# geonuklee/slam-toolkit

Hardware: NVIDIA B200
Metric: orb_extract_match_stereo_frames_per_s (higher is better)
Workload: dtype u8

## Files before the change

### slam-toolkit_b200/csrc/sfe_extract.cu

```cuda
#include <cuda_fp16.h>

#include <algorithm>
#include <cmath>
#include <mutex>
#include <type_traits>

#include "sfe_extract.cuh"

namespace sfe {

__device__ __forceinline__ uint32_t ldg_word_at(const uint8_t *p) {
    const uintptr_t a = (uintptr_t)p;
    const uint32_t *w = (const uint32_t *)(a & ~(uintptr_t)3);
    return __funnelshift_r(__ldg(w), __ldg(w + 1), (uint32_t)(a & 3) * 8);
}

__device__ __forceinline__ uint32_t dp4a_u8u8(uint32_t a, uint32_t b, uint32_t c) {
    uint32_t d;
    asm("dp4a.u32.u32 %0, %1, %2, %3;" : "=r"(d) : "r"(a), "r"(b), "r"(c));
    return d;
}
__device__ __forceinline__ uint32_t dp2a_lo(uint32_t a, uint32_t b, uint32_t c) {
    uint32_t d;
    asm("dp2a.lo.u32.u32 %0, %1, %2, %3;" : "=r"(d) : "r"(a), "r"(b), "r"(c));
// ... 892 lines not shown
        if (t.x0 == 0 || t.x0 + kBlurTileW + 3 > w) {
            for (int it = tid; it < IH * 6; it += 256) {
                const int r = (it * 10923) >> 16, k = it - r * 6;
                const int x = k < 3 ? k - 3 : w + (k - 3);
                const int c = x - x_first, sc = (k < 3 ? -x : 2 * w - 2 - x) - x_first;
                if (c >= 0 && c < IWW * 4 && sc >= 0) in8[r * IWW * 4 + c] = in8[r * IWW * 4 + sc];
            }
            __syncthreads();
        }
        if (t.y0 == 0 || t.y0 + kBlurTileH + 3 > h) {
            for (int it = tid; it < 6 * IWW; it += 256) {
                const int k = (it * (65536 / IWW + 1)) >> 16, j = it - k * IWW;
                const int y = k < 3 ? k - 3 : h + (k - 3);
                const int r = y - y_first, sr = (k < 3 ? -y : 2 * h - 2 - y) - y_first;
                if (r >= 0 && r < IH && sr >= 0) in32[r * IWW + j] = in32[sr * IWW + j];
            }
            __syncthreads();
        }
    } else {
        int pitch;
        const uint8_t *src = level_pixels(S, l, img, pitch);
        constexpr int kFirst = kBlurLead / 4 - 1, kWords = kBlurTileW / 4 + 2;
        for (int it = tid; it < IH * kWords; it += 256) {
            const int r = (it * (65536 / kWords + 1)) >> 16, j = kFirst + it - r * kWords;
            int yy = y_first + r;
            if ((unsigned)yy >= (unsigned)h) yy = reflect101(yy, h);
            const uint8_t *row = src + (size_t)yy * pitch;
            const int x = x_first + 4 * j;
            uint32_t v;
            if (x >= 0 && x + 8 <= w) {
                v = ldg_word_at(row + x);
            } else {
                v = __ldg(row + reflect101(x, w)) | (uint32_t)__ldg(row + reflect101(x + 1, w)) << 8 |
                    (uint32_t)__ldg(row + reflect101(x + 2, w)) << 16 | (uint32_t)__ldg(row + reflect101(x + 3, w)) << 24;
            }
            in32[r * IWW + j] = v;
        }
        __syncthreads();
    }
    constexpr uint32_t kTapLo = 18u | 34u << 8 | 48u << 16 | 56u << 24, kTapHi = 48u | 34u << 8 | 18u << 16;
    for (int it = tid; it < (IH / 2) * (kBlurTileW / 4); it += 256) {
        const int rp = it >> 5, g = it & 31;
        uint32_t hsum[2][4];
#pragma unroll
        for (int q = 0; q < 2; q++) {
            const uint32_t *wp = &in32[(2 * rp + q) * IWW + g + (kBlurLead / 4 - 1)];
            const uint32_t w0 = wp[0], w1 = wp[1], w2 = wp[2];
            hsum[q][0] = dp4a_u8u8(__byte_perm(w0, w1, 0x4321), kTapLo, dp4a_u8u8(__byte_perm(w1, w2, 0x4321), kTapHi, 0));
            hsum[q][1] = dp4a_u8u8(__byte_perm(w0, w1, 0x5432), kTapLo, dp4a_u8u8(__byte_perm(w1, w2, 0x5432), kTapHi, 0));
            hsum[q][2] = dp4a_u8u8(__byte_perm(w0, w1, 0x6543), kTapLo, dp4a_u8u8(__byte_perm(w1, w2, 0x6543), kTapHi, 0));
            hsum[q][3] = dp4a_u8u8(w1, kTapLo, dp4a_u8u8(w2, kTapHi, 0));
        }
        *(uint4 *)&hb[rp * kBlurTileW + 4 * g] =
            make_uint4(__byte_perm(hsum[0][0], hsum[1][0], 0x5410), __byte_perm(hsum[0][1], hsum[1][1], 0x5410),
                       __byte_perm(hsum[0][2], hsum[1][2], 0x5410), __byte_perm(hsum[0][3], hsum[1][3], 0x5410));
    }
    __syncthreads();
    uint8_t *dst = S.blur + (size_t)slot * S.blur_stride + L.blur_off;
    const int cg = tid & 31, r0 = (tid >> 5) * 4;
    const int gx = t.x0 + 4 * cg;
    if (gx >= w) return;
    uint4 pr[5];
#pragma unroll
    for (int p = 0; p < 5; p++) pr[p] = *(const uint4 *)&hb[(r0 / 2 + p) * kBlurTileW + 4 * cg];
    constexpr uint32_t kEvenA = 18u | 34u << 8 | 48u << 16 | 56u << 24, kEvenB = 48u | 34u << 8 | 18u << 16;
    constexpr uint32_t kOddA = 18u << 8 | 34u << 16 | 48u << 24, kOddB = 56u | 48u << 8 | 34u << 16 | 18u << 24;
#pragma unroll
    for (int k = 0; k < 4; k++) {
        const int gy = t.y0 + r0 + k;
        if (gy >= h) break;
        const int p = k >> 1;
        uint32_t v[4];
#pragma unroll
        for (int c = 0; c < 4; c++) {
            const uint32_t a0 = (&pr[p].x)[c], a1 = (&pr[p + 1].x)[c], a2 = (&pr[p + 2].x)[c], a3 = (&pr[p + 3].x)[c];
            v[c] = (k & 1) ? dp2a_hi(a3, kOddB, dp2a_lo(a2, kOddB, dp2a_hi(a1, kOddA, dp2a_lo(a0, kOddA, 32768u))))
                           : dp2a_hi(a3, kEvenB, dp2a_lo(a2, kEvenB, dp2a_hi(a1, kEvenA, dp2a_lo(a0, kEvenA, 32768u))));
        }
        *(uint32_t *)(dst + (size_t)gy * L.blur_pitch + gx) =
            __byte_perm(__byte_perm(v[0], v[1], 0x0062), __byte_perm(v[2], v[3], 0x0062), 0x5410);
    }
}

__device__ const signed char g_pattern[1024] = {
#include "orb_pattern_data.inc"
};

__device__ __forceinline__ float fast_atan2_deg(float y, float x) {
    constexpr float s = (float)(180.0 / 3.1415926535897932384626433832795);
    constexpr float p1 = 0.9997878412794807f * s, p3 = -0.3258083974640975f * s, p5 = 0.1555786518463281f * s,
                    p7 = -0.04432655554792128f * s;
    const float ax = fabsf(x), ay = fabsf(y);
    const float eps = 2.220446049250313e-16f;
    float a, c, c2;
    if (ax >= ay) {
        c = __fdiv_rn(ay, __fadd_rn(ax, eps));
        c2 = __fmul_rn(c, c);
        a = __fmul_rn(__fadd_rn(__fmul_rn(__fadd_rn(__fmul_rn(__fadd_rn(__fmul_rn(p7, c2), p5), c2), p3), c2), p1), c);
    } else {
        c = __fdiv_rn(ax, __fadd_rn(ay, eps));
        c2 = __fmul_rn(c, c);
        a = __fsub_rn(90.f, __fmul_rn(__fadd_rn(__fmul_rn(__fadd_rn(__fmul_rn(__fadd_rn(__fmul_rn(p7, c2), p5), c2), p3), c2), p1), c));
    }
    if (x < 0) a = __fsub_rn(180.f, a);
    if (y < 0) a = __fsub_rn(360.f, a);
    return a;
}

constexpr int kUmax[16] = {15, 15, 15, 15, 14, 14, 14, 13, 13, 12, 11, 10, 9, 8, 6, 3};
constexpr bool disc_is_symmetric() {
    for (int u = 0; u < 16; u++)
        for (int v = 0; v < 16; v++)
            if ((u <= kUmax[v]) != (v <= kUmax[u])) return false;
    return true;
}
static_assert(disc_is_symmetric(), "IC_Angle disc must be symmetric");
struct DiscTable {
    uint32_t u[16][8], in[16][8];
};
constexpr DiscTable make_disc_table() {
    DiscTable t{};
    for (int v = 0; v < 16; v++)
        for (int j = 0; j < 8; j++)
            for (int k = 0; k < 4; k++) {
                const int u = -kHalfPatch + 4 * j + k, au = u < 0 ? -u : u;
                if (au <= kUmax[v]) {
                    t.u[v][j] |= (uint32_t)(u & 0xFF) << (8 * k);
                    t.in[v][j] |= 1u << (8 * k);
                }
            }
    return t;
}
__device__ const DiscTable g_disc = make_disc_table();

__device__ __forceinline__ int dp4a_u8s8(uint32_t pix, uint32_t w, int acc) {
    int d;
    asm("dp4a.u32.s32 %0, %1, %2, %3;" : "=r"(d) : "r"(pix), "r"(w), "r"(acc));
    return d;
}

constexpr int kPatchR = 18;
constexpr int kPatchRows = 2 * kPatchR + 1, kPatchWords = 10;
constexpr signed char kPatternHost[1024] = {
#include "orb_pattern_data.inc"
};
constexpr bool pattern_within_patch() {
    for (int i = 0; i < 512; i++) {
        const int px = kPatternHost[2 * i], py = kPatternHost[2 * i + 1];
        if (4 * (px * px + py * py) >= (2 * kPatchR + 1) * (2 * kPatchR + 1)) return false;
    }
    return true;
}
static_assert(pattern_within_patch(), "a rotated pattern point could round outside the staged window");
#ifndef SFE_KP_PER_WARP
#define SFE_KP_PER_WARP 8
#endif
constexpr int kKpPerWarp = SFE_KP_PER_WARP;

constexpr int kIcBoxW = 48, kIcBoxH = 2 * kHalfPatch + 1, kBdBoxW = 64, kBdBoxH = kPatchRows;
constexpr int kIcBytes = 1536, kWinBytes = kIcBytes + 2432;
struct OrientMaps {
    CUtensorMap ic[kMaxLevels], ic_l0b;
    CUtensorMap bd[kMaxLevels];
};

template <bool kTma>
__global__ void __launch_bounds__(256, 5) orient_describe_kernel(ImgSet S, OutSet O, int kp_per_warp, const __grid_constant__ OrientMaps M) {
    __shared__ float2 pat[16 * 32];
    __shared__ __align__(128) uint8_t win_all[8][kTma ? kWinBytes : kPatchRows * kPatchWords * 4];
    __shared__ uint64_t bars[8];
    pdl_enter();
    const int tid = threadIdx.x, lane = tid & 31, warp = tid >> 5, img = blockIdx.y, slot = slot_of(S, img);
    uint32_t *patch = (uint32_t *)win_all[warp];
    uint32_t phase = 0;
    if (kTma && lane == 0) mbar_init(&bars[warp], 1);
    for (int i = tid; i < 512; i += 256) {
        const int byte = i >> 4, s = i & 15;
        pat[s * 32 + byte] = make_float2((float)g_pattern[2 * i], (float)g_pattern[2 * i + 1]);
    }
    const int wj = lane & 7, wr0 = 2 * (lane >> 3);
    auto ic_row = [wr0](int t) { return 8 * (t >> 1) + (t & 1) + wr0; };
    uint32_t wu[8], win[8];
#pragma unroll
    for (int t = 0; t < 8; t++) {
        const int r = ic_row(t), adv = r < 31 ? (r < kHalfPatch ? kHalfPatch - r : r - kHalfPatch) : 0;
        wu[t] = r < 31 ? __ldg(&g_disc.u[adv][wj]) : 0u;
        win[t] = r < 31 ? __ldg(&g_disc.in[adv][wj]) : 0u;
    }
    __syncthreads();
    const int cnt = lane < S.nlevels ? min(S.kp_count[slot * S.nlevels + lane], S.lv[lane].kp_cap) : 0;
    int inc = cnt;
#pragma unroll
    for (int o = 1; o < kMaxLevels; o <<= 1) {
        const int u = __shfl_up_sync(0xffffffffu, inc, o);
        if (lane >= o) inc += u;
    }
    const int total = __shfl_sync(0xffffffffu, inc, kMaxLevels - 1);
    const bool set_a = img < S.split;
    const int oi = set_a ? img : img - S.split;
    if (blockIdx.x == 0 && tid == 0) {
        (set_a ? O.n_a : O.n_b)[oi] = min(total, O.cap);
        if (total > O.cap) atomicOr(&S.flags[slot], kFlagOutOverflow);
    }
    const int g0 = (blockIdx.x * 8 + warp) * kp_per_warp;
    for (int g = g0; g < g0 + kp_per_warp; g++) {
        if (g >= total || g >= O.cap) return;
        const int l = __popc(__ballot_sync(0xffffffffu, lane < S.nlevels && inc <= g));
        const int local = g - __shfl_sync(0xffffffffu, inc - cnt, min(l, 31));
        const LevelPlan &L = S.lv[l];
        const uint32_t v = S.kpst[(size_t)slot * S.kpst_stride + L.kp_off + local];
        const int x = (v & 0xFFF) + kBorder, y = ((v >> 12) & 0xFFF) + kBorder;
        int pitch;
        const uint8_t *lvl = level_pixels(S, l, img, pitch);
        int m10 = 0, m01 = 0;
        const int xl = x - kPatchR, xb0 = xl & ~15;
        if (kTma) {
            const int xi = x - kHalfPatch, xi0 = xi & ~15;
            __syncwarp();
            if (lane == 0) {
                mbar_expect_tx(&bars[warp], kIcBoxW * kIcBoxH + kBdBoxW * kBdBoxH);
                const bool sa = img < S.split;
                const CUtensorMap *mi = l == 0 ? (sa ? &M.ic[0] : &M.ic_l0b) : &M.ic[l];
                tma_load_3d(win_all[warp], mi, &bars[warp], xi0, y - kHalfPatch, l == 0 ? S.in_z0 + (sa ? img : img - S.split) : slot);
                tma_load_3d(win_all[warp] + kIcBytes, &M.bd[l], &bars[warp], xb0, y - kPatchR, slot);
            }
            mbar_wait(&bars[warp], phase);
            phase ^= 1;
            const int o = xi - xi0;
            const uint32_t *w0 = (const uint32_t *)(win_all[warp] + (o & ~3) + 4 * wj);
            const uint32_t sh8 = (uint32_t)(o & 3) * 8;
#pragma unroll
            for (int t = 0; t < 8; t++) {
                const int r = ic_row(t);
                if (r < 31) {
                    const uint32_t *wp = w0 + r * (kIcBoxW / 4);
                    const uint32_t px = __funnelshift_r(wp[0], wp[1], sh8);
                    m10 = dp4a_u8s8(px, wu[t], m10);
                    m01 += (r - kHalfPatch) * dp4a_u8s8(px, win[t], 0);
                }
            }
        } else {
            const uint8_t *r0p = lvl + (size_t)(y - kHalfPatch) * pitch + (x - kHalfPatch + 4 * wj);
#pragma unroll
            for (int t = 0; t < 8; t++) {
                const int r = ic_row(t);
                if (r < 31) {
                    const uint8_t *rp = r0p + (size_t)r * pitch;
                    const uint32_t *wp = (const uint32_t *)((uintptr_t)rp & ~(uintptr_t)3);
                    const uint32_t px = __funnelshift_r(__ldg(wp), __ldg(wp + 1), ((uint32_t)(uintptr_t)rp & 3) * 8);
                    m10 = dp4a_u8s8(px, wu[t], m10);
                    m01 += (r - kHalfPatch) * dp4a_u8s8(px, win[t], 0);
                }
            }
        }
#pragma unroll
        for (int o = 16; o > 0; o >>= 1) {
            m01 += __shfl_xor_sync(0xffffffffu, m01, o);
            m10 += __shfl_xor_sync(0xffffffffu, m10, o);
        }
        const float angle = fast_atan2_deg((float)m01, (float)m10);
        float a = 0.f, b = 0.f;
        if (lane == 0) {
            const float factor_pi = (float)(3.1415926535897932384626433832795 / 180.0);
            const float rad = __fmul_rn(angle, factor_pi);
            double sn, cs;
            sincos((double)rad, &sn, &cs);
            a = (float)cs;
            b = (float)sn;
        }
        a = __shfl_sync(0xffffffffu, a, 0);
        b = __shfl_sync(0xffffffffu, b, 0);
        const uint8_t *pc;
        int wpitch;
        if (kTma) {
            wpitch = kBdBoxW;
            pc = win_all[warp] + kIcBytes + kPatchR * kBdBoxW + (xl - xb0) + kPatchR;
        } else {
            const int bp = L.blur_pitch;
            const uint8_t *bl = S.blur + (size_t)slot * S.blur_stride + L.blur_off;
            const int al = xl & 3;
            __syncwarp();
            if (lane < 3 * kPatchWords) {
                const int rs = lane / kPatchWords, c = lane - rs * kPatchWords;
                const uint32_t *src = (const uint32_t *)(bl + (size_t)(y - kPatchR + rs) * bp + (xl - al)) + c;
                uint32_t *dst = patch + rs * kPatchWords + c;
#pragma unroll
                for (int r = rs; r < kPatchRows; r += 3, src += 3 * (bp >> 2), dst += 3 * kPatchWords) *dst = __ldg(src);
            }
            __syncwarp();
            wpitch = kPatchWords * 4;
            pc = (const uint8_t *)patch + kPatchR * (kPatchWords * 4) + kPatchR + al;
        }
        uint32_t byte = 0;
#pragma unroll
        for (int k = 0; k < 8; k++) {
            int tv[2];
#pragma unroll
            for (int s = 0; s < 2; s++) {
                const float2 pp = pat[(2 * k + s) * 32 + lane];
                const int ry = __float2int_rn(__fadd_rn(__fmul_rn(pp.x, b), __fmul_rn(pp.y, a)));
                const int rx = __float2int_rn(__fsub_rn(__fmul_rn(pp.x, a), __fmul_rn(pp.y, b)));
                tv[s] = pc[ry * wpitch + rx];
            }
            byte |= (uint32_t)(tv[0] < tv[1]) << k;
        }
        uint8_t *desc = (set_a ? O.desc_a : O.desc_b) + ((size_t)oi * O.cap + g) * 32;
        desc[lane] = (uint8_t)byte;
        if (lane == 0) {
            sfe_keypoint kp;
            kp.x = (float)x;
            kp.y = (float)y;
            if (l != 0) {
                kp.x = __fmul_rn(kp.x, L.scale);
                kp.y = __fmul_rn(kp.y, L.scale);
            }
            kp.size = L.size;
            kp.angle = angle;
            kp.response = (float)(v >> 24);
            kp.octave = l;
            kp.class_id = -1;
            (set_a ? O.kps_a : O.kps_b)[(size_t)oi * O.cap + g] = kp;
        }
    }
}

}

using namespace sfe;

enum { kStagePyramid, kStageFast, kStageQuadtree, kStageBlur, kStageDescribe, kStageStereo, kStageTrack, kNumStages };
constexpr int kOctreeSmemCand = 3072;
constexpr int kComputeStreams = 4;
constexpr int kMaxChunks = 16;

struct sfe_extractor {
    int device = 0;
    cudaStream_t stream = nullptr;
    cudaStream_t s_h2d = nullptr, s_d2h = nullptr;
    cudaStream_t extra[kComputeStreams - 1] = {};
    int n_compute = 3;
    cudaStream_t aux[3] = {nullptr, nullptr, nullptr};
    cudaEvent_t ev_fork[3] = {}, ev_join[3] = {};
    int dev_split = 3;
    bool split_small = false;
    int octree_ctas = 0;
    int sm_count = 148;
    bool piped_now = false;
    bool orient_tma = true;
    bool overlap_tail = true;
    bool tail_pending = false;
    int overlap_blur = 2;
    cudaEvent_t ev_start = nullptr;
    bool async_dev = false;
    cudaEvent_t ev_in[kMaxChunks] = {}, ev_done[kMaxChunks] = {};
    int chunks_override = 0;
    bool trace = false;
    cudaEvent_t tr_ev[3 * kMaxChunks + 1] = {};
    sfe_extractor_params prm{};
    float scale[kMaxLevels], inv_scale[kMaxLevels], sigma2[kMaxLevels], inv_sigma2[kMaxLevels];
    int quota[kMaxLevels];
    int max_images = 0;
    int w = 0, h = 0;
    LevelPlan lv[kMaxLevels];
    FastPlan fast{};
    alignas(64) TmaMaps fast_maps{}, blur_maps{}, pyr_maps{};
    alignas(64) OrientMaps orient_maps{};
    int pyr_box_w = 0, pyr_box_h = 0;
    bool tma_plan_ok = false, tma_disabled = false, tma_now = false;
    const void *l0_key[2] = {nullptr, nullptr};
    size_t l0_geom[4] = {0, 0, 0, 0};
    int pitch0 = 0;
    std::vector<SegRec> segs;
    int seg_level_start[kMaxLevels + 1] = {};
    DevBuf<SegRec> d_segs;
    size_t fast_smem = 0, pyr_smem = 0;
    int pyr_wide_h[kMaxLevels] = {};
    std::vector<TilePlan> tiles;
    size_t pyr_stride = 0, blur_stride = 0;
    int cand_stride = 0, kpst_stride = 0, max_cand = 0, max_nodes = 0;
    size_t octree_smem = 0;
    int octree_smem_cand = 0, octree_slots = 0, octree_cand_override = 0;
    struct GraphEntry {
        uint64_t plan_gen = 0;
        int frames = 0, cap = 0, stereo = 0, seen = 0;
        double sp[3] = {0, 0, 0};
        const void *ptr[7] = {};
        cudaGraphExec_t exec = nullptr;
        int64_t launches = 0;
        uint64_t used = 0;
    };
    std::vector<GraphEntry> graphs;
    uint64_t plan_gen = 0, graph_clock = 0;
    bool use_graphs = true;
    bool use_pdl = true;
    bool octree_ff = true;
    bool pdl_now = false;
    bool octree_wide = false;
    int cand_floor[kMaxLevels] = {};
    int cand_cap_override = 0;
    DevBuf<uint8_t> d_octree_scratch;
    DevBuf<uint8_t> d_pyr, d_blur, d_in, d_l0, d_desc;
    DevBuf<uint32_t> d_cand, d_kpst;
    DevBuf<int> d_counts;
    DevBuf<TilePlan> d_tiles;
    DevBuf<uint2> d_xtab, d_ytab;
    DevBuf<sfe_keypoint> d_kps;
    DevBuf<int32_t> d_nout, d_sidx, d_sdist, d_tidx, d_tdist;
    std::vector<int> h_flags;
    int *h_flags_pinned = nullptr;
    uint8_t *h_stage = nullptr;
    size_t h_stage_bytes = 0;
    bool use_copy_kernel = true;
    int64_t launches = 0;
    bool profiling = false;
    cudaEvent_t prof_ev[kNumStages + 1] = {};
    bool prof_pending = false, prof_has_stereo = false, prof_has_track = false;
    TrackScratch track;
    double stage_ms[kNumStages] = {};
    int64_t stage_calls = 0;
    ImgSet last{};
    int last_count = 0;
};

static inline int cv_round_f(float v) { return (int)nearbyintf(v); }

static inline void prof_mark(sfe_extractor *ex, int i) {
    if (ex->profiling) cudaEventRecord(ex->prof_ev[i], ex->stream);
}

static void build_tables(sfe_extractor *ex) {
    const int nl = ex->prm.nlevels;
// ... 422 lines not shown
            SFE_CUDA(cudaFuncSetAttribute(octree_kernel<false>, cudaFuncAttributeMaxDynamicSharedMemorySize, (int)ex->octree_smem));
            SFE_CUDA(cudaFuncSetAttribute(octree_kernel<true>, cudaFuncAttributeMaxDynamicSharedMemorySize, (int)ex->octree_smem));
            granted[ex->device & 63] = ex->octree_smem;
        }
    }
    int *scratch_next = ex->d_counts.p + (size_t)ex->max_images * nl * 2;
    auto launch_octree = [&](cudaStream_t so, int level0, int level_n, int ctas) {
        const int items = level_n * count;
        const int grid = ctas > 0 ? std::min(items, ctas) : items;
        const int threads = nl * count <= ex->sm_count / 2 ? 1024 : 256;
        if (ex->octree_wide)
            launch_k(octree_kernel<true>, grid, threads, ex->octree_smem, so, ex->pdl_now, S, count, level0, level_n, ex->octree_smem_cand,
                     ex->max_cand, ex->max_nodes, ex->d_octree_scratch.p, ex->octree_slots, scratch_next);
        else
            launch_k(octree_kernel<false>, grid, threads, ex->octree_smem, so, ex->pdl_now, S, count, level0, level_n, ex->octree_smem_cand,
                     ex->max_cand, ex->max_nodes, ex->d_octree_scratch.p, ex->octree_slots, scratch_next);
        ex->launches++;
    };
    const bool fork_ok = !ex->profiling && !ex->piped_now && st == ex->stream;
    const bool split = fork_ok && has_cells && ex->split_small && count <= kSplitMaxImages && nl >= 3;
    if (split) {
        launch_pyr(1);
        cudaStream_t sa = ex->aux[2];
        SFE_CUDA(cudaEventRecord(ex->ev_fork[2], st));
        SFE_CUDA(cudaStreamWaitEvent(sa, ex->ev_fork[2], 0));
        if (int rc = launch_fast(ex, sa, S, count, 0, 2)) return rc;
        launch_octree(sa, 0, 2, 0);
        SFE_CUDA(cudaEventRecord(ex->ev_join[2], sa));
        for (int l = 2; l < nl; l++) launch_pyr(l);
        cudaStream_t sb = ex->aux[0];
        SFE_CUDA(cudaEventRecord(ex->ev_fork[0], st));
        SFE_CUDA(cudaStreamWaitEvent(sb, ex->ev_fork[0], 0));
        if (ex->tma_now)
            blur_kernel<true><<<dim3((unsigned)ex->tiles.size(), count), 256, 0, sb>>>(S, ex->d_tiles.p, ex->blur_maps);
        else
            blur_kernel<false><<<dim3((unsigned)ex->tiles.size(), count), 256, 0, sb>>>(S, ex->d_tiles.p, ex->blur_maps);
        SFE_CUDA(cudaEventRecord(ex->ev_join[0], sb));
        if (int rc = launch_fast(ex, st, S, count, 2, nl)) return rc;
        launch_octree(st, 2, nl - 2, 0);
        SFE_CUDA(cudaStreamWaitEvent(st, ex->ev_join[2], 0));
        SFE_CUDA(cudaStreamWaitEvent(st, ex->ev_join[0], 0));
        ex->launches += 3;
    } else {
        for (int l = 1; l < nl; l++) launch_pyr(l);
        prof_mark(ex, 1);
        if (has_cells) {
            const int si = 0;
            const bool fork = ex->overlap_blur && fork_ok, late = ex->overlap_blur == 2;
            cudaStream_t sb = fork ? ex->aux[si] : st;
            auto launch_blur = [&]() {
                if (ex->tma_now)
                    blur_kernel<true><<<dim3((unsigned)ex->tiles.size(), count), 256, 0, sb>>>(S, ex->d_tiles.p, ex->blur_maps);
                else
                    blur_kernel<false><<<dim3((unsigned)ex->tiles.size(), count), 256, 0, sb>>>(S, ex->d_tiles.p, ex->blur_maps);
            };
            auto fork_blur = [&]() -> int {
                SFE_CUDA(cudaEventRecord(ex->ev_fork[si], st));
                SFE_CUDA(cudaStreamWaitEvent(sb, ex->ev_fork[si], 0));
                launch_blur();
                SFE_CUDA(cudaEventRecord(ex->ev_join[si], sb));
                return SFE_OK;
            };
            if (fork && !late)
                if (int rc = fork_blur()) return rc;
            if (int rc = launch_fast(ex, st, S, count)) return rc;
            prof_mark(ex, 2);
            if (fork && late)
                if (int rc = fork_blur()) return rc;
            launch_octree(st, 0, nl, ex->octree_ctas > 0 ? ex->octree_ctas : (fork && late ? 2 * ex->sm_count : 0));
            prof_mark(ex, 3);
            if (fork) SFE_CUDA(cudaStreamWaitEvent(st, ex->ev_join[si], 0));
            else launch_blur();
            prof_mark(ex, 4);
            ex->launches += 2;
        } else {
            prof_mark(ex, 2); prof_mark(ex, 3); prof_mark(ex, 4);
        }
    }
    if (st == ex->stream) {
        if (int rc = join_tail(ex)) return rc;
    } else if (ex->tail_pending) {
        SFE_CUDA(cudaStreamWaitEvent(st, ex->ev_join[1], 0));
    }
    const int kpw = std::max(1, std::min(kKpPerWarp, div_up(O.cap * count, ex->sm_count * 5 * 8)));
    if (ex->tma_now && ex->orient_tma)
        launch_k(orient_describe_kernel<true>, dim3(div_up(O.cap, 8 * kpw), count), 256, 0, st, ex->pdl_now, S, O, kpw, ex->orient_maps);
    else
        launch_k(orient_describe_kernel<false>, dim3(div_up(O.cap, 8 * kpw), count), 256, 0, st, ex->pdl_now, S, O, kpw, ex->orient_maps);
    prof_mark(ex, 5);
    ex->prof_pending = ex->profiling;
    ex->prof_has_stereo = ex->prof_has_track = false;
    ex->launches++;
    SFE_CUDA(cudaGetLastError());
    return SFE_OK;
}

constexpr int kStatusRerun = -1000;

static int grow_candidate_buffers(sfe_extractor *ex, int count) {
    const int nl = ex->prm.nlevels;
    std::vector<int> cnt((size_t)count * nl);
    SFE_CUDA(cudaMemcpy(cnt.data(), ex->d_counts.p, sizeof(int) * cnt.size(), cudaMemcpyDeviceToHost));
    bool grew = false;
    for (int l = 0; l < nl; l++) {
        int most = 0, who = 0;
        for (int i = 0; i < count; i++)
            if (cnt[(size_t)i * nl + l] > most) { most = cnt[(size_t)i * nl + l]; who = i; }
        if (most <= ex->lv[l].cand_cap) continue;
        if (most > kMaxCandCap) {
            set_error("image slot %d, level %d: %d FAST corners, more than the %d a level may hold", who, l, most, kMaxCandCap);
            return SFE_ERR_CAPACITY;
        }
        ex->cand_floor[l] = std::min(kMaxCandCap, most + most / 8 + 64);
        grew = true;
    }
    if (!grew)
        for (int l = 0; l < nl; l++) {
            if (ex->lv[l].cand_cap >= kMaxCandCap) continue;
            ex->cand_floor[l] = std::min(kMaxCandCap, 2 * std::max(ex->lv[l].cand_cap, 1024));
            grew = true;
        }
    if (!grew) { set_error("FAST candidate buffers are at their maximum (%d per level)", kMaxCandCap); return SFE_ERR_CAPACITY; }
    if (ex->tail_pending) { cudaStreamSynchronize(ex->aux[1]); ex->tail_pending = false; }
    ex->w = ex->h = 0;
    ex->last_count = 0;
    return kStatusRerun;
}

static int check_flags(sfe_extractor *ex, cudaStream_t st, int count, bool flags_here = false) {
    ex->h_flags.resize(count);
    if (!flags_here) SFE_CUDA(cudaMemcpyAsync(ex->h_flags.data(), ex->last.flags, sizeof(int) * count, cudaMemcpyDeviceToHost, st));
    SFE_CUDA(cudaStreamSynchronize(st));
    if (flags_here) memcpy(ex->h_flags.data(), ex->h_flags_pinned, sizeof(int) * count);
    if (ex->prof_pending) {
        const int ns = ex->prof_has_track ? kNumStages : ex->prof_has_stereo ? kNumStages - 1 : kNumStages - 2;
        for (int i = 0; i < ns; i++) {
            float ms = 0.f;
            if (cudaEventElapsedTime(&ms, ex->prof_ev[i], ex->prof_ev[i + 1]) == cudaSuccess) ex->stage_ms[i] += ms;
        }
        ex->stage_calls++;
        ex->prof_pending = false;
    }
    bool cand = false;
    for (int i = 0; i < count; i++) {
        if (ex->h_flags[i] & kFlagNodeOverflow) { set_error("image %d: quadtree node buffer overflow", i); return SFE_ERR_CAPACITY; }
        cand = cand || (ex->h_flags[i] & kFlagCandOverflow);
    }
    if (cand) return grow_candidate_buffers(ex, count);
    for (int i = 0; i < count; i++)
        if (ex->h_flags[i] & kFlagOutOverflow) { set_error("image %d: more keypoints than the caller's capacity", i); return SFE_ERR_CAPACITY; }
    return SFE_OK;
}

static int finish_dev(sfe_extractor *ex, int count) {
    if (ex->async_dev) return SFE_OK;
    return check_flags(ex, ex->stream, count);
}

static int prepare(sfe_extractor *ex, int count, int w, int h, int stride, int cap) {
    SFE_REQUIRE(ex != nullptr, SFE_ERR_BAD_ARG, "null handle");
    SFE_REQUIRE(count >= 1 && count <= ex->max_images, SFE_ERR_BAD_ARG, "count outside [1, max_images]");
    SFE_REQUIRE(w > 0 && h > 0 && stride >= w, SFE_ERR_BAD_ARG, "bad image geometry");
    SFE_REQUIRE(cap >= 1 && cap < 65536, SFE_ERR_BAD_ARG, "capacity must be in [1, 65535]");
    if (w != ex->w || h != ex->h) {
        if (ex->tail_pending) SFE_CUDA(cudaStreamSynchronize(ex->aux[1]));
        int rc = build_plan(ex, w, h);
        if (rc != SFE_OK) { ex->w = ex->h = 0; return rc; }
// ... 275 lines not shown
        const double e = now_us();
        const double d[6] = {tr_t[1] - tr_t[0], tr_t[2] - tr_t[1], tr_t[3] - tr_t[2], tr_t[4] - tr_t[3], tr_t[5] - tr_t[4], e - tr_t[5]};
        for (int i = 0; i < 6; i++) tr_acc[i] += d[i];
        if (++tr_n % 100 == 0) {
            fprintf(stderr, "sfe small-call trace (us, mean of 100): enqueue upload %.1f | upload done %.1f | enqueue kernels %.1f | kernels done %.1f | enqueue downloads %.1f | downloads done %.1f\n",
                    tr_acc[0] / 100, tr_acc[1] / 100, tr_acc[2] / 100, tr_acc[3] / 100, tr_acc[4] / 100, tr_acc[5] / 100);
            for (double &a : tr_acc) a = 0;
        }
    }
    if (ex->trace) {
        fprintf(stderr, "sfe trace: %d frames in %d sub-batches (ms since the first upload was queued)\n", frames, nch);
        for (int c = 0; c < nch; c++) {
            float a = 0, b = 0, d = 0;
            cudaEventElapsedTime(&a, ex->tr_ev[3 * kMaxChunks], ex->tr_ev[3 * c]);
            cudaEventElapsedTime(&b, ex->tr_ev[3 * kMaxChunks], ex->tr_ev[3 * c + 1]);
            cudaEventElapsedTime(&d, ex->tr_ev[3 * kMaxChunks], ex->tr_ev[3 * c + 2]);
            fprintf(stderr, "  sub-batch %2d frames [%3d,%3d): uploaded %.3f  computed %.3f  downloaded %.3f\n", c, bound[c], bound[c + 1], a, b, d);
        }
    }
    return rc;
}

static int run_host_batch(sfe_extractor *ex, const uint8_t *left, const uint8_t *right, size_t image_stride, int frames, int w,
                          int h, int stride, const sfe_stereo_params *sp, sfe_keypoint *kps_l, uint8_t *desc_l, int32_t *n_l,
                          sfe_keypoint *kps_r, uint8_t *desc_r, int32_t *n_r, int32_t *stereo_idx, int32_t *stereo_dist,
                          int cap, const sfe_track_params *tp = nullptr, int32_t *track_idx = nullptr,
                          int32_t *track_dist = nullptr) {
    int rc = kStatusRerun;
    for (int attempt = 0; attempt < 3 && rc == kStatusRerun; attempt++)
        rc = run_host_batch_once(ex, left, right, image_stride, frames, w, h, stride, sp, kps_l, desc_l, n_l, kps_r, desc_r, n_r,
                                 stereo_idx, stereo_dist, cap, tp, track_idx, track_dist);
    if (rc == kStatusRerun) { set_error("FAST candidate buffers still overflow after two re-runs"); rc = SFE_ERR_CAPACITY; }
    return rc;
}

extern "C" {

int sfe_extractor_create(const sfe_extractor_params *p, int device, int max_images, sfe_extractor **out) {
    SFE_REQUIRE(p && out, SFE_ERR_BAD_ARG, "null argument");
    SFE_REQUIRE(p->nlevels >= 1 && p->nlevels <= kMaxLevels, SFE_ERR_BAD_ARG, "nlevels outside [1,16]");
    SFE_REQUIRE(p->nfeatures >= 1 && p->nfeatures <= 60000, SFE_ERR_BAD_ARG, "nfeatures outside [1,60000]");
    SFE_REQUIRE(p->scale_factor > 1.0f, SFE_ERR_BAD_ARG, "scale_factor must be > 1");
    SFE_REQUIRE(p->ini_th_fast >= 1 && p->min_th_fast >= 1 && p->ini_th_fast < 255 && p->min_th_fast < 255, SFE_ERR_BAD_ARG,
                "FAST thresholds outside [1,254]");
    SFE_REQUIRE(max_images >= 1 && max_images <= 65535, SFE_ERR_BAD_ARG, "max_images outside [1,65535]");
    int ndev = 0;
    SFE_CUDA(cudaGetDeviceCount(&ndev));
    SFE_REQUIRE(ndev > 0, SFE_ERR_NO_DEVICE, "no CUDA device (there is no CPU fallback)");
    SFE_REQUIRE(device >= 0 && device < ndev, SFE_ERR_BAD_ARG, "device index out of range");
    DeviceGuard g(device);
    SFE_REQUIRE(g.ok, SFE_ERR_NO_DEVICE, "cannot select the handle's device");
    sfe_extractor *ex = new sfe_extractor();
    ex->device = device;
    ex->prm = *p;
    ex->max_images = max_images;
    cudaError_t e = cudaStreamCreateWithFlags(&ex->stream, cudaStreamNonBlocking);
    if (e != cudaSuccess) {
        set_error("cudaStreamCreate: %s", cudaGetErrorString(e));
        delete ex;
        return SFE_ERR_CUDA;
    }
    bool ok = cudaStreamCreateWithFlags(&ex->s_h2d, cudaStreamNonBlocking) == cudaSuccess &&
              cudaStreamCreateWithFlags(&ex->s_d2h, cudaStreamNonBlocking) == cudaSuccess &&
              cudaEventCreateWithFlags(&ex->ev_start, cudaEventDisableTiming) == cudaSuccess;
    for (int i = 0; i < kComputeStreams - 1 && ok; i++) ok = cudaStreamCreateWithFlags(&ex->extra[i], cudaStreamNonBlocking) == cudaSuccess;
    for (int i = 0; i < 3 && ok; i++)
        ok = cudaStreamCreateWithFlags(&ex->aux[i], cudaStreamNonBlocking) == cudaSuccess &&
             cudaEventCreateWithFlags(&ex->ev_fork[i], cudaEventDisableTiming) == cudaSuccess &&
             cudaEventCreateWithFlags(&ex->ev_join[i], cudaEventDisableTiming) == cudaSuccess;
    for (int i = 0; i < kMaxChunks && ok; i++)
        ok = cudaEventCreateWithFlags(&ex->ev_in[i], cudaEventDisableTiming) == cudaSuccess &&
             cudaEventCreateWithFlags(&ex->ev_done[i], cudaEventDisableTiming) == cudaSuccess;
    if (!ok) {
        set_error("stream/event creation: %s", cudaGetErrorString(cudaGetLastError()));
        sfe_extractor_destroy(ex);
        return SFE_ERR_CUDA;
    }
    if (const char *env = getenv("SFE_PIPELINE_CHUNKS")) ex->chunks_override = atoi(env);
    if (const char *env = getenv("SFE_NO_TMA")) ex->tma_disabled = atoi(env) != 0;
    if (const char *env = getenv("SFE_OVERLAP_BLUR")) ex->overlap_blur = atoi(env);
    cudaDeviceGetAttribute(&ex->sm_count, cudaDevAttrMultiProcessorCount, device);
    if (const char *env = getenv("SFE_OCTREE_CTAS")) ex->octree_ctas = atoi(env);
    if (const char *env = getenv("SFE_ORIENT_TMA")) ex->orient_tma = atoi(env) != 0;
    if (const char *env = getenv("SFE_OVERLAP_TAIL")) ex->overlap_tail = atoi(env) != 0;
    if (const char *env = getenv("SFE_TRACE")) ex->trace = atoi(env) != 0;
    if (const char *env = getenv("SFE_COMPUTE_STREAMS")) ex->n_compute = std::max(1, std::min(atoi(env), kComputeStreams));
    if (ex->trace)
        for (auto &e : ex->tr_ev) cudaEventCreate(&e);
    if (const char *env = getenv("SFE_OCTREE_SMEM_CAND")) ex->octree_cand_override = atoi(env);
    if (const char *env = getenv("SFE_CAND_CAP")) ex->cand_cap_override = std::max(8, atoi(env));
    if (const char *env = getenv("SFE_GRAPHS")) ex->use_graphs = atoi(env) != 0;
    if (const char *env = getenv("SFE_PDL")) ex->use_pdl = atoi(env) != 0;
    if (const char *env = getenv("SFE_OCTREE_FF")) ex->octree_ff = atoi(env) != 0;
    if (const char *env = getenv("SFE_COPY_KERNEL")) ex->use_copy_kernel = atoi(env) != 0;
    if (const char *env = getenv("SFE_SPLIT_SMALL")) ex->split_small = atoi(env) != 0;
    if (const char *env = getenv("SFE_DEV_SPLIT")) ex->dev_split = std::max(1, std::min(atoi(env), kComputeStreams));
    build_tables(ex);
    *out = ex;
    return SFE_OK;
}

int sfe_extractor_destroy(sfe_extractor *ex) {
    if (!ex) return SFE_OK;
    drop_graphs(ex);
    if (ex->h_flags_pinned) cudaFreeHost(ex->h_flags_pinned);
    if (ex->h_stage) cudaFreeHost(ex->h_stage);
    DeviceGuard g(ex->device);
    SFE_REQUIRE(g.ok, SFE_ERR_NO_DEVICE, "cannot select the handle's device");
    cudaStreamSynchronize(ex->stream);
    ex->d_pyr.release(); ex->d_blur.release(); ex->d_in.release(); ex->d_l0.release(); ex->d_octree_scratch.release(); ex->d_desc.release();
    ex->d_cand.release(); ex->d_kpst.release(); ex->d_counts.release();
    ex->d_tiles.release(); ex->d_segs.release(); ex->d_xtab.release(); ex->d_ytab.release();
    ex->d_kps.release(); ex->d_nout.release(); ex->d_sidx.release(); ex->d_sdist.release(); ex->d_tidx.release(); ex->d_tdist.release();
    ex->track.cell_start.release(); ex->track.order.release(); ex->track.valid.release(); ex->track.sxy.release(); ex->track.sdesc.release(); ex->track.best.release();
    for (int i = 0; i <= kNumStages; i++)
        if (ex->prof_ev[i]) cudaEventDestroy(ex->prof_ev[i]);
    for (int i = 0; i < kMaxChunks; i++) {
        if (ex->ev_in[i]) cudaEventDestroy(ex->ev_in[i]);
        if (ex->ev_done[i]) cudaEventDestroy(ex->ev_done[i]);
    }
    for (auto &e : ex->tr_ev)
        if (e) cudaEventDestroy(e);
    for (int i = 0; i < 3; i++) {
        if (ex->ev_fork[i]) cudaEventDestroy(ex->ev_fork[i]);
        if (ex->ev_join[i]) cudaEventDestroy(ex->ev_join[i]);
        if (ex->aux[i]) cudaStreamDestroy(ex->aux[i]);
    }
    if (ex->ev_start) cudaEventDestroy(ex->ev_start);
    for (auto &e : ex->extra)
        if (e) cudaStreamDestroy(e);
    if (ex->s_h2d) cudaStreamDestroy(ex->s_h2d);
    if (ex->s_d2h) cudaStreamDestroy(ex->s_d2h);
    cudaStreamDestroy(ex->stream);
    delete ex;
    return SFE_OK;
}

int sfe_extractor_tables(const sfe_extractor *ex, float *scale, float *inv_scale, float *sigma2, float *inv_sigma2,
                         int32_t *per_level) {
    SFE_REQUIRE(ex, SFE_ERR_BAD_ARG, "null handle");
    for (int i = 0; i < ex->prm.nlevels; i++) {
        if (scale) scale[i] = ex->scale[i];
        if (inv_scale) inv_scale[i] = ex->inv_scale[i];
        if (sigma2) sigma2[i] = ex->sigma2[i];
        if (inv_sigma2) inv_sigma2[i] = ex->inv_sigma2[i];
        if (per_level) per_level[i] = ex->quota[i];
    }
    return SFE_OK;
}

int sfe_extractor_level_size(const sfe_extractor *ex, int w, int h, int level, int *lw, int *lh) {
    SFE_REQUIRE(ex && lw && lh && level >= 0 && level < ex->prm.nlevels, SFE_ERR_BAD_ARG, "bad argument");
    *lw = cv_round_f((float)w * ex->inv_scale[level]);
    *lh = cv_round_f((float)h * ex->inv_scale[level]);
    return SFE_OK;
}

int sfe_extractor_max_keypoints_for(const sfe_extractor *ex, int w, int h, int *cap) {
    SFE_REQUIRE(ex && cap, SFE_ERR_BAD_ARG, "null argument");
    int total = 0;
    for (int l = 0; l < ex->prm.nlevels; l++) {
        int n_ini = 4;
        if (w > 0 && h > 0) {
            const int ww = cv_round_f((float)w * ex->inv_scale[l]) - 2 * kBorder, wh = cv_round_f((float)h * ex->inv_scale[l]) - 2 * kBorder;
            n_ini = ww > 0 && wh > 0 ? std::max(1, (int)roundf((float)ww / (float)wh)) : 1;
        }
// ... 355 lines not shown
```

Baseline: 68200.

## Pipeline orient/describe TMA loads with double buffers and batch per-lane keypoint setup

Restructures the orient/describe kernel so each warp resolves all its keypoints up front, one per lane, then double-buffers TMA loads of the intensity-centroid and BRIEF windows. The next window is prefetched while the current one is processed, which hides the serial per-keypoint load latency. Angle/sincos and keypoint writes now run in parallel across lanes instead of only on lane 0. The pattern is read into registers instead of a shared table, and rounding uses a magic-number add with raw ld.shared, removing the prologue __syncthreads. In exchange the kernel uses more shared memory, the launch bound drops to 4 blocks per SM, and a runtime kp_per_warp override is added.

```diff
diff --git a/slam-toolkit_b200/csrc/sfe_extract.cu b/slam-toolkit_b200/csrc/sfe_extract.cu
--- a/slam-toolkit_b200/csrc/sfe_extract.cu
+++ b/slam-toolkit_b200/csrc/sfe_extract.cu
@@ -998,7 +998,7 @@
     }
 }
 
-__device__ const signed char g_pattern[1024] = {
+__device__ __align__(16) const signed char g_pattern[1024] = {
 #include "orb_pattern_data.inc"
 };
 
@@ -1068,42 +1068,30 @@
     return true;
 }
 static_assert(pattern_within_patch(), "a rotated pattern point could round outside the staged window");
-#ifndef SFE_KP_PER_WARP
-#define SFE_KP_PER_WARP 8
-#endif
-constexpr int kKpPerWarp = SFE_KP_PER_WARP;
+constexpr int kKpPerWarp = 8;
 
 constexpr int kIcBoxW = 48, kIcBoxH = 2 * kHalfPatch + 1, kBdBoxW = 64, kBdBoxH = kPatchRows;
-constexpr int kIcBytes = 1536, kWinBytes = kIcBytes + 2432;
+constexpr int kBufBytes = 2432;
+static_assert(kBdBoxW * kBdBoxH <= kBufBytes && kIcBoxW * kIcBoxH <= kBufBytes && kBufBytes % 128 == 0, "window buffer size");
 struct OrientMaps {
     CUtensorMap ic[kMaxLevels], ic_l0b;
     CUtensorMap bd[kMaxLevels];
 };
+constexpr float kRoundMagic = 12582912.f;
+constexpr uint32_t kRoundBias = 0x4B400000u;
+__device__ __forceinline__ int lds_u8(uint32_t addr) {
+    uint32_t v;
+    asm volatile("ld.shared.u8 %0, [%1];" : "=r"(v) : "r"(addr));
+    return (int)v;
+}
 
 template <bool kTma>
-__global__ void __launch_bounds__(256, 5) orient_describe_kernel(ImgSet S, OutSet O, int kp_per_warp, const __grid_constant__ OrientMaps M) {
-    __shared__ float2 pat[16 * 32];
-    __shared__ __align__(128) uint8_t win_all[8][kTma ? kWinBytes : kPatchRows * kPatchWords * 4];
-    __shared__ uint64_t bars[8];
+__global__ void __launch_bounds__(256, 4) orient_describe_kernel(ImgSet S, OutSet O, int kp_per_warp, const __grid_constant__ OrientMaps M) {
+    constexpr int kBuf = kTma ? kBufBytes : kPatchRows * kPatchWords * 4;
+    __shared__ __align__(128) uint8_t win_all[8][kTma ? 2 : 1][kBuf];
+    __shared__ uint64_t bars[8][2];
     pdl_enter();
     const int tid = threadIdx.x, lane = tid & 31, warp = tid >> 5, img = blockIdx.y, slot = slot_of(S, img);
-    uint32_t *patch = (uint32_t *)win_all[warp];
-    uint32_t phase = 0;
-    if (kTma && lane == 0) mbar_init(&bars[warp], 1);
-    for (int i = tid; i < 512; i += 256) {
-        const int byte = i >> 4, s = i & 15;
-        pat[s * 32 + byte] = make_float2((float)g_pattern[2 * i], (float)g_pattern[2 * i + 1]);
-    }
-    const int wj = lane & 7, wr0 = 2 * (lane >> 3);
-    auto ic_row = [wr0](int t) { return 8 * (t >> 1) + (t & 1) + wr0; };
-    uint32_t wu[8], win[8];
-#pragma unroll
-    for (int t = 0; t < 8; t++) {
-        const int r = ic_row(t), adv = r < 31 ? (r < kHalfPatch ? kHalfPatch - r : r - kHalfPatch) : 0;
-        wu[t] = r < 31 ? __ldg(&g_disc.u[adv][wj]) : 0u;
-        win[t] = r < 31 ? __ldg(&g_disc.in[adv][wj]) : 0u;
-    }
-    __syncthreads();
     const int cnt = lane < S.nlevels ? min(S.kp_count[slot * S.nlevels + lane], S.lv[lane].kp_cap) : 0;
     int inc = cnt;
 #pragma unroll
@@ -1119,93 +1107,167 @@
         if (total > O.cap) atomicOr(&S.flags[slot], kFlagOutOverflow);
     }
     const int g0 = (blockIdx.x * 8 + warp) * kp_per_warp;
-    for (int g = g0; g < g0 + kp_per_warp; g++) {
-        if (g >= total || g >= O.cap) return;
-        const int l = __popc(__ballot_sync(0xffffffffu, lane < S.nlevels && inc <= g));
-        const int local = g - __shfl_sync(0xffffffffu, inc - cnt, min(l, 31));
-        const LevelPlan &L = S.lv[l];
-        const uint32_t v = S.kpst[(size_t)slot * S.kpst_stride + L.kp_off + local];
-        const int x = (v & 0xFFF) + kBorder, y = ((v >> 12) & 0xFFF) + kBorder;
-        int pitch;
-        const uint8_t *lvl = level_pixels(S, l, img, pitch);
-        int m10 = 0, m01 = 0;
-        const int xl = x - kPatchR, xb0 = xl & ~15;
+    const int nb = min(kp_per_warp, min(total, O.cap) - g0);
+    if (nb <= 0) return;
+
+    const bool own = lane < nb;
+    const int g = g0 + lane;
+    int l = 0;
+#pragma unroll
+    for (int k = 0; k < kMaxLevels; k++) {
+        const int p = __shfl_sync(0xffffffffu, inc, k);
+        l += (k < S.nlevels && p <= g);
+    }
+    const int first = __shfl_sync(0xffffffffu, inc - cnt, min(l, 31));
+    if (!own) l = 0;
+    const LevelPlan &L = S.lv[l];
+    const uint32_t v = own ? S.kpst[(size_t)slot * S.kpst_stride + L.kp_off + (g - first)] : 0u;
+    const int x = (v & 0xFFF) + kBorder, y = ((v >> 12) & 0xFFF) + kBorder;
+    const int xl = x - kPatchR;
+    uint32_t phase = 0;
+    if (kTma && lane < 2) mbar_init(&bars[warp][lane], 1);
+    __syncwarp();
+    const bool sa = img < S.split;
+    auto issue_ic = [&](int j, int buf) {
+        if (lane == j) {
+            const CUtensorMap *mi = l == 0 ? (sa ? &M.ic[0] : &M.ic_l0b) : &M.ic[l];
+            mbar_expect_tx(&bars[warp][buf], kIcBoxW * kIcBoxH);
+            tma_load_3d(win_all[warp][buf], mi, &bars[warp][buf], (x - kHalfPatch) & ~15, y - kHalfPatch,
+                        l == 0 ? S.in_z0 + (sa ? img : img - S.split) : slot);
+        }
+    };
+    auto issue_bd = [&](int j, int buf) {
+        if (lane == j) {
+            mbar_expect_tx(&bars[warp][buf], kBdBoxW * kBdBoxH);
+            tma_load_3d(win_all[warp][buf], &M.bd[l], &bars[warp][buf], xl & ~15, y - kPatchR, slot);
+        }
+    };
+    auto wait_buf = [&](int buf) {
+        mbar_wait(&bars[warp][buf], (phase >> buf) & 1);
+        phase ^= 1u << buf;
+    };
+
+    int M01 = 0, M10 = 0;
+    {
+        const int wj = lane & 7, wr0 = 2 * (lane >> 3);
+        auto ic_row = [wr0](int t) { return 8 * (t >> 1) + (t & 1) + wr0; };
+        uint32_t wu[8], win[8];
+#pragma unroll
+        for (int t = 0; t < 8; t++) {
+            const int r = ic_row(t), adv = r < 31 ? (r < kHalfPatch ? kHalfPatch - r : r - kHalfPatch) : 0;
+            wu[t] = r < 31 ? __ldg(&g_disc.u[adv][wj]) : 0u;
+            win[t] = r < 31 ? __ldg(&g_disc.in[adv][wj]) : 0u;
+        }
+        int pitch = 0;
+        const uint8_t *lvl = kTma ? nullptr : level_pixels(S, l, img, pitch);
         if (kTma) {
-            const int xi = x - kHalfPatch, xi0 = xi & ~15;
+            issue_ic(0, nb & 1);
+            if (nb == 1) issue_bd(0, 0);
+        }
+        for (int j = 0; j < nb; j++) {
+            int m10 = 0, m01 = 0;
+            if (kTma) {
+                const int buf = (j + nb) & 1;
+                if (j + 1 < nb) issue_ic(j + 1, buf ^ 1);
+                const int o = __shfl_sync(0xffffffffu, (x - kHalfPatch) & 15, j);
+                wait_buf(buf);
+                const uint32_t *w0 = (const uint32_t *)(win_all[warp][buf] + (o & ~3) + 4 * wj);
+                const uint32_t sh8 = (uint32_t)(o & 3) * 8;
+#pragma unroll
+                for (int t = 0; t < 8; t++) {
+                    const int r = ic_row(t);
+                    if (r < 31) {
+                        const uint32_t *wp = w0 + r * (kIcBoxW / 4);
+                        const uint32_t px = __funnelshift_r(wp[0], wp[1], sh8);
+                        m10 = dp4a_u8s8(px, wu[t], m10);
+                        m01 += (r - kHalfPatch) * dp4a_u8s8(px, win[t], 0);
+                    }
+                }
+            } else {
+                const uint8_t *r0p = (const uint8_t *)__shfl_sync(0xffffffffu, (unsigned long long)(lvl + (size_t)(y - kHalfPatch) * pitch + (x - kHalfPatch)), j) + 4 * wj;
+                const int pj = __shfl_sync(0xffffffffu, pitch, j);
+#pragma unroll
+                for (int t = 0; t < 8; t++) {
+                    const int r = ic_row(t);
+                    if (r < 31) {
+                        const uint8_t *rp = r0p + (size_t)r * pj;
+                        const uint32_t *wp = (const uint32_t *)((uintptr_t)rp & ~(uintptr_t)3);
+                        const uint32_t px = __funnelshift_r(__ldg(wp), __ldg(wp + 1), ((uint32_t)(uintptr_t)rp & 3) * 8);
+                        m10 = dp4a_u8s8(px, wu[t], m10);
+                        m01 += (r - kHalfPatch) * dp4a_u8s8(px, win[t], 0);
+                    }
+                }
+            }
+#pragma unroll
+            for (int o = 16; o > 0; o >>= 1) {
+                m01 += __shfl_xor_sync(0xffffffffu, m01, o);
+                m10 += __shfl_xor_sync(0xffffffffu, m10, o);
+            }
+            if (lane == j) {
+                M01 = m01;
+                M10 = m10;
+            }
             __syncwarp();
-            if (lane == 0) {
-                mbar_expect_tx(&bars[warp], kIcBoxW * kIcBoxH + kBdBoxW * kBdBoxH);
-                const bool sa = img < S.split;
-                const CUtensorMap *mi = l == 0 ? (sa ? &M.ic[0] : &M.ic_l0b) : &M.ic[l];
-                tma_load_3d(win_all[warp], mi, &bars[warp], xi0, y - kHalfPatch, l == 0 ? S.in_z0 + (sa ? img : img - S.split) : slot);
-                tma_load_3d(win_all[warp] + kIcBytes, &M.bd[l], &bars[warp], xb0, y - kPatchR, slot);
-            }
-            mbar_wait(&bars[warp], phase);
-            phase ^= 1;
-            const int o = xi - xi0;
-            const uint32_t *w0 = (const uint32_t *)(win_all[warp] + (o & ~3) + 4 * wj);
-            const uint32_t sh8 = (uint32_t)(o & 3) * 8;
-#pragma unroll
-            for (int t = 0; t < 8; t++) {
-                const int r = ic_row(t);
-                if (r < 31) {
-                    const uint32_t *wp = w0 + r * (kIcBoxW / 4);
-                    const uint32_t px = __funnelshift_r(wp[0], wp[1], sh8);
-                    m10 = dp4a_u8s8(px, wu[t], m10);
-                    m01 += (r - kHalfPatch) * dp4a_u8s8(px, win[t], 0);
-                }
-            }
+            if (kTma && j == nb - 2) issue_bd(0, 0);
+        }
+    }
+    if (kTma && nb > 1) issue_bd(1, 1);
+
+    float ca = 0.f, sb = 0.f;
+    if (own) {
+        const float angle = fast_atan2_deg((float)M01, (float)M10);
+        const float factor_pi = (float)(3.1415926535897932384626433832795 / 180.0);
+        const float rad = __fmul_rn(angle, factor_pi);
+        double sn, cs;
+        sincos((double)rad, &sn, &cs);
+        ca = (float)cs;
+        sb = (float)sn;
+        sfe_keypoint kp;
+        kp.x = (float)x;
+        kp.y = (float)y;
+        if (l != 0) {
+            kp.x = __fmul_rn(kp.x, L.scale);
+            kp.y = __fmul_rn(kp.y, L.scale);
+        }
+        kp.size = L.size;
+        kp.angle = angle;
+        kp.response = (float)(v >> 24);
+        kp.octave = l;
+        kp.class_id = -1;
+        (set_a ? O.kps_a : O.kps_b)[(size_t)oi * O.cap + g] = kp;
+    }
+
+    constexpr int wpitch = kTma ? kBdBoxW : kPatchWords * 4;
+    const uint32_t boff = (uint32_t)(kPatchR * wpitch + kPatchR + (kTma ? (xl & 15) : (xl & 3))) - kRoundBias * (uint32_t)(wpitch + 1);
+    float px[16], py[16];
+    {
+        const int4 *pp = (const int4 *)(g_pattern + 32 * lane);
+        const int4 p0 = __ldg(pp), p1 = __ldg(pp + 1);
+        const int w[8] = {p0.x, p0.y, p0.z, p0.w, p1.x, p1.y, p1.z, p1.w};
+#pragma unroll
+        for (int s = 0; s < 16; s++) {
+            px[s] = (float)(signed char)(w[s >> 1] >> (16 * (s & 1)));
+            py[s] = (float)(signed char)(w[s >> 1] >> (16 * (s & 1) + 8));
+        }
+    }
+    const uint8_t *bl = kTma ? nullptr : S.blur + (size_t)slot * S.blur_stride + L.blur_off + (size_t)(y - kPatchR) * L.blur_pitch + (xl & ~3);
+    for (int j = 0; j < nb; j++) {
+        const float a = __shfl_sync(0xffffffffu, ca, j), b = __shfl_sync(0xffffffffu, sb, j);
+        const int buf = kTma ? j & 1 : 0;
+        const uint32_t base = smem_u32(win_all[warp][buf]) + __shfl_sync(0xffffffffu, boff, j);
+        if (kTma) {
+            wait_buf(buf);
         } else {
-            const uint8_t *r0p = lvl + (size_t)(y - kHalfPatch) * pitch + (x - kHalfPatch + 4 * wj);
-#pragma unroll
-            for (int t = 0; t < 8; t++) {
-                const int r = ic_row(t);
-                if (r < 31) {
-                    const uint8_t *rp = r0p + (size_t)r * pitch;
-                    const uint32_t *wp = (const uint32_t *)((uintptr_t)rp & ~(uintptr_t)3);
-                    const uint32_t px = __funnelshift_r(__ldg(wp), __ldg(wp + 1), ((uint32_t)(uintptr_t)rp & 3) * 8);
-                    m10 = dp4a_u8s8(px, wu[t], m10);
-                    m01 += (r - kHalfPatch) * dp4a_u8s8(px, win[t], 0);
-                }
-            }
-        }
-#pragma unroll
-        for (int o = 16; o > 0; o >>= 1) {
-            m01 += __shfl_xor_sync(0xffffffffu, m01, o);
-            m10 += __shfl_xor_sync(0xffffffffu, m10, o);
-        }
-        const float angle = fast_atan2_deg((float)m01, (float)m10);
-        float a = 0.f, b = 0.f;
-        if (lane == 0) {
-            const float factor_pi = (float)(3.1415926535897932384626433832795 / 180.0);
-            const float rad = __fmul_rn(angle, factor_pi);
-            double sn, cs;
-            sincos((double)rad, &sn, &cs);
-            a = (float)cs;
-            b = (float)sn;
-        }
-        a = __shfl_sync(0xffffffffu, a, 0);
-        b = __shfl_sync(0xffffffffu, b, 0);
-        const uint8_t *pc;
-        int wpitch;
-        if (kTma) {
-            wpitch = kBdBoxW;
-            pc = win_all[warp] + kIcBytes + kPatchR * kBdBoxW + (xl - xb0) + kPatchR;
-        } else {
-            const int bp = L.blur_pitch;
-            const uint8_t *bl = S.blur + (size_t)slot * S.blur_stride + L.blur_off;
-            const int al = xl & 3;
-            __syncwarp();
+            const uint8_t *src0 = (const uint8_t *)__shfl_sync(0xffffffffu, (unsigned long long)bl, j);
+            const int bp = __shfl_sync(0xffffffffu, (int)L.blur_pitch, j);
             if (lane < 3 * kPatchWords) {
                 const int rs = lane / kPatchWords, c = lane - rs * kPatchWords;
-                const uint32_t *src = (const uint32_t *)(bl + (size_t)(y - kPatchR + rs) * bp + (xl - al)) + c;
-                uint32_t *dst = patch + rs * kPatchWords + c;
+                const uint32_t *src = (const uint32_t *)(src0 + (size_t)rs * bp) + c;
+                uint32_t *dst = (uint32_t *)win_all[warp][0] + rs * kPatchWords + c;
 #pragma unroll
                 for (int r = rs; r < kPatchRows; r += 3, src += 3 * (bp >> 2), dst += 3 * kPatchWords) *dst = __ldg(src);
             }
             __syncwarp();
-            wpitch = kPatchWords * 4;
-            pc = (const uint8_t *)patch + kPatchR * (kPatchWords * 4) + kPatchR + al;
         }
         uint32_t byte = 0;
 #pragma unroll
@@ -1213,30 +1275,17 @@
             int tv[2];
 #pragma unroll
             for (int s = 0; s < 2; s++) {
-                const float2 pp = pat[(2 * k + s) * 32 + lane];
-                const int ry = __float2int_rn(__fadd_rn(__fmul_rn(pp.x, b), __fmul_rn(pp.y, a)));
-                const int rx = __float2int_rn(__fsub_rn(__fmul_rn(pp.x, a), __fmul_rn(pp.y, b)));
-                tv[s] = pc[ry * wpitch + rx];
+                const int i = 2 * k + s;
+                const float fy = __fadd_rn(__fadd_rn(__fmul_rn(px[i], b), __fmul_rn(py[i], a)), kRoundMagic);
+                const float fx = __fadd_rn(__fsub_rn(__fmul_rn(px[i], a), __fmul_rn(py[i], b)), kRoundMagic);
+                tv[s] = lds_u8(base + __float_as_uint(fy) * (uint32_t)wpitch + __float_as_uint(fx));
             }
             byte |= (uint32_t)(tv[0] < tv[1]) << k;
         }
-        uint8_t *desc = (set_a ? O.desc_a : O.desc_b) + ((size_t)oi * O.cap + g) * 32;
+        uint8_t *desc = (set_a ? O.desc_a : O.desc_b) + ((size_t)oi * O.cap + g0 + j) * 32;
         desc[lane] = (uint8_t)byte;
-        if (lane == 0) {
-            sfe_keypoint kp;
-            kp.x = (float)x;
-            kp.y = (float)y;
-            if (l != 0) {
-                kp.x = __fmul_rn(kp.x, L.scale);
-                kp.y = __fmul_rn(kp.y, L.scale);
-            }
-            kp.size = L.size;
-            kp.angle = angle;
-            kp.response = (float)(v >> 24);
-            kp.octave = l;
-            kp.class_id = -1;
-            (set_a ? O.kps_a : O.kps_b)[(size_t)oi * O.cap + g] = kp;
-        }
+        __syncwarp();
+        if (kTma && j + 2 < nb) issue_bd(j + 2, buf);
     }
 }
 
@@ -1263,6 +1312,7 @@
     int sm_count = 148;
     bool piped_now = false;
     bool orient_tma = true;
+    int kp_per_warp = 0;
     bool overlap_tail = true;
     bool tail_pending = false;
     int overlap_blur = 2;
@@ -1851,7 +1901,7 @@
     } else if (ex->tail_pending) {
         SFE_CUDA(cudaStreamWaitEvent(st, ex->ev_join[1], 0));
     }
-    const int kpw = std::max(1, std::min(kKpPerWarp, div_up(O.cap * count, ex->sm_count * 5 * 8)));
+    const int kpw = ex->kp_per_warp > 0 ? ex->kp_per_warp : std::max(1, std::min(kKpPerWarp, div_up(O.cap * count, ex->sm_count * 5 * 8)));
     if (ex->tma_now && ex->orient_tma)
         launch_k(orient_describe_kernel<true>, dim3(div_up(O.cap, 8 * kpw), count), 256, 0, st, ex->pdl_now, S, O, kpw, ex->orient_maps);
     else
@@ -2293,6 +2343,7 @@
     cudaDeviceGetAttribute(&ex->sm_count, cudaDevAttrMultiProcessorCount, device);
     if (const char *env = getenv("SFE_OCTREE_CTAS")) ex->octree_ctas = atoi(env);
     if (const char *env = getenv("SFE_ORIENT_TMA")) ex->orient_tma = atoi(env) != 0;
+    if (const char *env = getenv("SFE_KP_PER_WARP")) ex->kp_per_warp = std::max(1, std::min(atoi(env), 32));
     if (const char *env = getenv("SFE_OVERLAP_TAIL")) ex->overlap_tail = atoi(env) != 0;
     if (const char *env = getenv("SFE_TRACE")) ex->trace = atoi(env) != 0;
     if (const char *env = getenv("SFE_COMPUTE_STREAMS")) ex->n_compute = std::max(1, std::min(atoi(env), kComputeStreams));
```

After: 68610 (median of 6 runs). About the same (+0.6%).
